# lucidrains/nuwa-pytorch

Hardware: AMD Instinct MI355X
Metric: video-tokens/sec, 3DNA decoder fwd+bwd @ 10x16x16 (higher is better)
Workload: dtype bf16/fp16 operands, fp32 accumulate -- forward: 3-MFMA bf16 hi+lo pairs on cross-attention kv projection, to_logits; 2 fp16 MFMAs (fp16 activation x fp16 hi+lo weight) on to_out x2, cross-attention q projection; single fp16 MFMA on 3DNA q/k/v projection, FF1 + gate, FF2, Sparse3DNA core, cross-atten

## Files before the change

nuwa_pytorch_amd/csrc/elementwise.hip:

```cpp
#include "common.h"
#include "../../include/amdnuwa.h"

namespace {

constexpr int MAXV = 4;
constexpr int ROWS_PER_BLOCK = 4;

template <int NV> struct RowValsT { float4 v[NV]; };
typedef RowValsT<MAXV> RowVals;

template <bool BF>
__device__ __forceinline__ float4 ld4(const void* base, size_t i) {
    if (BF) {
        const uint2 v = *reinterpret_cast<const uint2*>(reinterpret_cast<const bf16_t*>(base) + i);
        return make_float4(__uint_as_float(v.x << 16), __uint_as_float(v.x & 0xffff0000u), __uint_as_float(v.y << 16), __uint_as_float(v.y & 0xffff0000u));
    }
    return *reinterpret_cast<const float4*>(reinterpret_cast<const float*>(base) + i);
}
__device__ __forceinline__ float4 ld4h(const void* base, size_t i) {
    const uint2 v = *reinterpret_cast<const uint2*>(reinterpret_cast<const uint16_t*>(base) + i);
    return make_float4(f16lo_f(v.x), f16hi_f(v.x), f16lo_f(v.y), f16hi_f(v.y));
}
template <int FMT>
__device__ __forceinline__ float4 ld4f(const void* base, size_t i) {
    if constexpr (FMT == 2) return ld4h(base, i);
    else return ld4<FMT == 1>(base, i);
}
template <int FMT, int NV>
__device__ __forceinline__ void row_load_f(const void* base, size_t row_off, int D, int lane, RowValsT<NV>& r, float mul = 1.f) {
#pragma unroll
    for (int it = 0; it < NV; ++it) {
        const int e = (lane + it * 64) * 4;
        const bool in = e < D;
        const float4 v = ld4f<FMT>(base, row_off + (in ? e : 0));
        r.v[it] = make_float4(in ? v.x * mul : 0.f, in ? v.y * mul : 0.f, in ? v.z * mul : 0.f, in ? v.w * mul : 0.f);
    }
}
template <bool BF, int NV>
__device__ __forceinline__ void row_load_t(const void* base, size_t row_off, int D, int lane, RowValsT<NV>& r, float fill = 0.f) {
#pragma unroll
    for (int it = 0; it < NV; ++it) {
        const int e = (lane + it * 64) * 4;
        const bool in = e < D;
        const float4 v = ld4<BF>(base, row_off + (in ? e : 0));
        r.v[it] = make_float4(in ? v.x : fill, in ? v.y : fill, in ? v.z : fill, in ? v.w : fill);
    }
}

typedef float f32x4v __attribute__((ext_vector_type(4)));
typedef uint32_t u32x2v __attribute__((ext_vector_type(2)));
template <bool BF>
__device__ __forceinline__ float4 ld4_nt(const void* base, size_t i) {
    if (BF) {
        const u32x2v v = __builtin_nontemporal_load(reinterpret_cast<const u32x2v*>(reinterpret_cast<const bf16_t*>(base) + i));
        return make_float4(__uint_as_float(v.x << 16), __uint_as_float(v.x & 0xffff0000u), __uint_as_float(v.y << 16), __uint_as_float(v.y & 0xffff0000u));
    }
    const f32x4v v = __builtin_nontemporal_load(reinterpret_cast<const f32x4v*>(reinterpret_cast<const float*>(base) + i));
    return make_float4(v.x, v.y, v.z, v.w);
}
__device__ __forceinline__ void st4_nt(float* p, float4 v) {
    const f32x4v t = {v.x, v.y, v.z, v.w};
    __builtin_nontemporal_store(t, reinterpret_cast<f32x4v*>(p));
}
__device__ __forceinline__ void st_bf16x4_nt(bf16_t* p, float a, float b, float c, float d) {
    const u32x2v t = {pack2_rne(a, b), pack2_rne(c, d)};
    __builtin_nontemporal_store(t, reinterpret_cast<u32x2v*>(p));
}

template <int NV>
__device__ __forceinline__ void row_load(const float* __restrict__ p, int D, int lane, RowValsT<NV>& r, float fill = 0.f) {
#pragma unroll
    for (int it = 0; it < NV; ++it) {
        const int e = (lane + it * 64) * 4;
        const bool in = e < D;
        const float4 v = *reinterpret_cast<const float4*>(p + (in ? e : 0));
        r.v[it] = make_float4(in ? v.x : fill, in ? v.y : fill, in ? v.z : fill, in ? v.w : fill);
    }
}
__device__ __forceinline__ float4 ldp4(const float* __restrict__ p, int e, int D) {
    const bool in = e < D;
    const float4 v = *reinterpret_cast<const float4*>(p + (in ? e : 0));
    return make_float4(in ? v.x : 0.f, in ? v.y : 0.f, in ? v.z : 0.f, in ? v.w : 0.f);
}
__device__ __forceinline__ void store_bf16x4(bf16_t* hi, bf16_t* lo, int e, float a, float b, float c, float d, int lo_f16 = 0, float* sat = nullptr) {
    float dummy = 0.f;
    float& mx = sat ? *sat : dummy;
    if (lo_f16 == 2) { *reinterpret_cast<uint2*>(hi + e) = make_uint2(pack2_f16_sat_n(a, b, mx), pack2_f16_sat_n(c, d, mx)); return; }
    if (!lo) { *reinterpret_cast<uint2*>(hi + e) = make_uint2(pack2_rne(a, b), pack2_rne(c, d)); return; }
    if (lo_f16) {
        *reinterpret_cast<uint2*>(hi + e) = make_uint2(pack2_rne(a, b), pack2_rne(c, d));
        *reinterpret_cast<uint2*>(lo + e) = make_uint2(pack2_f16_sat_n(a, b, mx), pack2_f16_sat_n(c, d, mx));
        return;
    }
    bf16_t h[4], l[4];
    f2bf_hilo(a, h[0], l[0]); f2bf_hilo(b, h[1], l[1]); f2bf_hilo(c, h[2], l[2]); f2bf_hilo(d, h[3], l[3]);
    *reinterpret_cast<uint2*>(hi + e) = make_uint2(pack2(h[0], h[1]), pack2(h[2], h[3]));
    if (lo) *reinterpret_cast<uint2*>(lo + e) = make_uint2(pack2(l[0], l[1]), pack2(l[2], l[3]));
}

__device__ __forceinline__ void store_ln_shifted(bf16_t* out_hi, bf16_t* out_lo, long long row, int e, int D, int shift_ntok,
                                                 int shift_fmap, float y0, float y1, float y2, float y3, int lo_f16 = 0, float* sat = nullptr) {
    long long drow = row;
    bool keep = true, zero_own = false;
    if (shift_ntok > 0 && shift_fmap < 0) {
        const int i = (int)(row % shift_ntok);
        if (e < (D >> 1)) { keep = i + 1 < shift_ntok; drow = row + 1; zero_own = i == 0; }
    } else if (shift_ntok > 0) {
        const int i = (int)(row % shift_ntok);
        const int qd = e < (D >> 2) ? 0 : (e < (D >> 1) ? 1 : 2);
        if (i > 0 && qd < 2) {
            const int p = i - 1, wq = p % shift_fmap, yq = (p / shift_fmap) % shift_fmap;
            if (qd == 0) { keep = yq + 1 < shift_fmap && i + shift_fmap < shift_ntok; drow = row + shift_fmap; zero_own = yq == 0; }
            else         { keep = wq + 1 < shift_fmap && i + 1 < shift_ntok;          drow = row + 1;          zero_own = wq == 0; }
        }
    }
    if (keep) store_bf16x4(out_hi + drow * D, out_lo ? out_lo + drow * D : nullptr, e, y0, y1, y2, y3, lo_f16, sat);
    if (zero_own) store_bf16x4(out_hi + row * D, out_lo ? out_lo + row * D : nullptr, e, 0.f, 0.f, 0.f, 0.f, lo_f16, sat);
}

template <int NV>
__device__ __forceinline__ void row_mean_rstd(const RowValsT<NV>& xv, int D, int lane, float eps, float& mean, float& rstd) {
// ... 189 lines not shown
            const float4 wv = ldp4(w, e, D);
            float4 xx = cur.xv.v[it];
            const float4 gg = cur.gv.v[it];
            if (STABLE) { xx.x *= ia; xx.y *= ia; xx.z *= ia; xx.w *= ia; }
            xh[it] = make_float4((xx.x - mean) * rstd, (xx.y - mean) * rstd, (xx.z - mean) * rstd, (xx.w - mean) * rstd);
            g[it] = make_float4(gg.x * wv.x, gg.y * wv.y, gg.z * wv.z, gg.w * wv.w);
            s1 += (g[it].x + g[it].y) + (g[it].z + g[it].w);
            s2 += (g[it].x * xh[it].x + g[it].y * xh[it].y) + (g[it].z * xh[it].z + g[it].w * xh[it].w);
            pw[it].x += gg.x * xh[it].x; pw[it].y += gg.y * xh[it].y; pw[it].z += gg.z * xh[it].z; pw[it].w += gg.w * xh[it].w;
            pb[it].x += gg.x; pb[it].y += gg.y; pb[it].z += gg.z; pb[it].w += gg.w;
        }
        const float m1 = wave_sum(s1) / D, m2 = wave_sum(s2) / D;
        const float sc = STABLE ? rstd * ia : rstd;
#pragma unroll
        for (int it = 0; it < NV; ++it) {
            const int e = (lane + it * 64) * 4;
            if (e >= D) continue;
            const float d0 = sc * (g[it].x - m1 - xh[it].x * m2), d1 = sc * (g[it].y - m1 - xh[it].y * m2);
            const float d2 = sc * (g[it].z - m1 - xh[it].z * m2), d3 = sc * (g[it].w - m1 - xh[it].w * m2);
            ps[it].x += d0; ps[it].y += d1; ps[it].z += d2; ps[it].w += d3;
            if (OUT == 0) {
                if (out_f16) store_bf16x4(dx_hi + row * D, nullptr, e, d0 * gout, d1 * gout, d2 * gout, d3 * gout, 2, &sat);
                else store_bf16x4(dx_hi + row * D, dx_lo ? dx_lo + row * D : nullptr, e, d0, d1, d2, d3);
            } else {
                const float4 o = cur.rv.v[it];
                *reinterpret_cast<float4*>(dx_acc + row * D + e) = make_float4(o.x + d0, o.y + d1, o.z + d2, o.w + d3);
            }
        }
    };
    for (; row < R; row += 2 * stride) {
        const bool m1 = row + stride < R;
        if (m1) load_row(row + stride, bufB);
        process(bufA, row);
        if (!m1) break;
        if (row + 2 * stride < R) load_row(row + 2 * stride, bufA);
        process(bufB, row + stride);
    }
    if (OUT == 0) f16_sat_commit(sat);
#pragma unroll
    for (int it = 0; it < NV; ++it) {
        const int e = (lane + it * 64) * 4;
        *reinterpret_cast<float4*>(&red[wv_][0][e]) = pw[it];
        *reinterpret_cast<float4*>(&red[wv_][1][e]) = pb[it];
        *reinterpret_cast<float4*>(&red[wv_][2][e]) = ps[it];
    }
    __syncthreads();
    for (int idx = threadIdx.x; idx < 3 * D; idx += 256) {
        const int k = idx / D, c = idx % D;
        partial[((size_t)blockIdx.x * 3 + k) * D + c] = ((red[0][k][c] + red[1][k][c]) + red[2][k][c]) + red[3][k][c];
    }
}

template <int NV, int BFM, int NT = 0>
__global__ __launch_bounds__(256) void ln_bwd_chain_kernel(const float* __restrict__ dh, const float* __restrict__ x,
                                                           const float* __restrict__ mean_i, const float* __restrict__ rstd_i,
                                                           const float* __restrict__ w, const float* __restrict__ gres,
                                                           float* __restrict__ dx_out, const float* __restrict__ yprev,
                                                           const float* __restrict__ meanp_i, const float* __restrict__ rstdp_i,
                                                           const float* __restrict__ wprev, bf16_t* __restrict__ dyp_hi,
                                                           bf16_t* __restrict__ dyp_lo, float* __restrict__ partA,
                                                           float* __restrict__ partB, long long R, int D, int shift_ntok,
                                                           int shift_fmap, const float* __restrict__ scale2, int out_f16) {
#pragma clang fp contract(off)
    constexpr bool BF = BFM == 1 || BFM == 2, YBF = BFM == 1;
    constexpr int DHF = BFM == 3 ? 2 : (BF ? 1 : 0);
    const float gin = BFM == 3 ? f16_gs_inv(scale2) : 1.f, gout = out_f16 ? f16_gs(scale2) : 1.f;
    float sat = 0.f;
    __shared__ float red[ROWS_PER_BLOCK][3][NV * 256];
    const int lane = threadIdx.x & 63, wv_ = __builtin_amdgcn_readfirstlane(threadIdx.x >> 6);
    float4 pwA[NV], pbA[NV], pwB[NV], pbB[NV], psB[NV];
#pragma unroll
    for (int it = 0; it < NV; ++it) pwA[it] = pbA[it] = pwB[it] = pbB[it] = psB[it] = make_float4(0.f, 0.f, 0.f, 0.f);
    const int quarter = D >> 2;
    const float4 zero4 = make_float4(0.f, 0.f, 0.f, 0.f);
    struct RowIn { RowValsT<NV> xv, gv, rv, yv; float mean, rstd, meanp, rstdp; };
    auto load_row = [&](long long row, RowIn& in) {
        if (NT & 2) {
#pragma unroll
            for (int it = 0; it < NV; ++it) { const int e = (lane + it * 64) * 4; in.xv.v[it] = e < D ? ld4_nt<false>(x, (size_t)row * D + e) : zero4; }
        } else row_load(x + row * D, D, lane, in.xv);
        if (shift_ntok > 0) {
            const int i = (int)(row % shift_ntok);
            long long src_h = -1, src_w = -1;
            const bool audio = shift_fmap < 0;
            if (audio) {
                if (i + 1 < shift_ntok) src_h = src_w = row + 1;
            } else if (i > 0) {
                const int p = i - 1, wq = p % shift_fmap, yq = (p / shift_fmap) % shift_fmap;
                if (yq < shift_fmap - 1 && i + shift_fmap < shift_ntok) src_h = row + shift_fmap;
                if (wq < shift_fmap - 1 && i + 1 < shift_ntok) src_w = row + 1;
            }
#pragma unroll
            for (int it = 0; it < NV; ++it) {
                const int e0 = (lane + it * 64) * 4;
                const bool inr = e0 < D;
                const int e = inr ? e0 : 0;
                long long src = row;
                if (i > 0 || audio) { if (e < quarter) src = src_h; else if (e < 2 * quarter) src = src_w; }
                const bool has = src >= 0 && inr;
                const size_t so = (size_t)(has ? src : row) * D + e;
                const float4 v = BFM == 3 ? ld4h(dh, so) : ((NT & 2) ? ld4_nt<BF>(dh, so) : ld4<BF>(dh, so));
                in.gv.v[it] = make_float4(has ? v.x : 0.f, has ? v.y : 0.f, has ? v.z : 0.f, has ? v.w : 0.f);
            }
        } else {
            if (BFM == 3) row_load_f<2>(dh, (size_t)row * D, D, lane, in.gv);
            else row_load_t<BF>(dh, (size_t)row * D, D, lane, in.gv);
        }
        if (NT & 2) {
#pragma unroll
            for (int it = 0; it < NV; ++it) {
                const int e = (lane + it * 64) * 4;
                in.rv.v[it] = e < D ? ld4_nt<false>(gres, (size_t)row * D + e) : zero4;
                in.yv.v[it] = e < D ? ld4_nt<YBF>(yprev, (size_t)row * D + e) : zero4;
            }
        } else {
            row_load(gres + row * D, D, lane, in.rv);
            row_load_t<YBF>(yprev, (size_t)row * D, D, lane, in.yv);
        }
        in.mean = mean_i[row]; in.rstd = rstd_i[row]; in.meanp = meanp_i[row]; in.rstdp = rstdp_i[row];
    };
    const long long stride = (long long)gridDim.x * ROWS_PER_BLOCK;
    long long row = (long long)blockIdx.x * ROWS_PER_BLOCK + wv_;
    RowIn bufA, bufB;
    if (row < R) load_row(row, bufA);
    auto process = [&](const RowIn& cur, long long row) {
        float s1 = 0.f, s2 = 0.f;
        float4 xh[NV], g[NV];
#pragma unroll
        for (int it = 0; it < NV; ++it) {
            const int e = (lane + it * 64) * 4;
            const float4 wv = ldp4(w, e, D);
            const float4 xx = cur.xv.v[it], gg = cur.gv.v[it];
            xh[it] = make_float4((xx.x - cur.mean) * cur.rstd, (xx.y - cur.mean) * cur.rstd, (xx.z - cur.mean) * cur.rstd, (xx.w - cur.mean) * cur.rstd);
            g[it] = make_float4(gg.x * wv.x, gg.y * wv.y, gg.z * wv.z, gg.w * wv.w);
            s1 += (g[it].x + g[it].y) + (g[it].z + g[it].w);
            s2 += (g[it].x * xh[it].x + g[it].y * xh[it].y) + (g[it].z * xh[it].z + g[it].w * xh[it].w);
            pwA[it].x += gg.x * xh[it].x; pwA[it].y += gg.y * xh[it].y; pwA[it].z += gg.z * xh[it].z; pwA[it].w += gg.w * xh[it].w;
            pbA[it].x += gg.x; pbA[it].y += gg.y; pbA[it].z += gg.z; pbA[it].w += gg.w;
        }
        const float m1 = wave_sum(s1) / D, m2 = wave_sum(s2) / D;
        float4 dx[NV];
#pragma unroll
        for (int it = 0; it < NV; ++it) {
            const int e = (lane + it * 64) * 4;
            if (e >= D) { dx[it] = zero4; continue; }
            const float4 o = cur.rv.v[it];
            const float rs = BFM == 3 ? cur.rstd * gin : cur.rstd;
            dx[it] = make_float4(o.x + rs * (g[it].x - m1 - xh[it].x * m2), o.y + rs * (g[it].y - m1 - xh[it].y * m2),
                                 o.z + rs * (g[it].z - m1 - xh[it].z * m2), o.w + rs * (g[it].w - m1 - xh[it].w * m2));
            if (NT & 1) st4_nt(dx_out + row * D + e, dx[it]); else *reinterpret_cast<float4*>(dx_out + row * D + e) = dx[it];
        }
        s1 = 0.f; s2 = 0.f;
#pragma unroll
        for (int it = 0; it < NV; ++it) {
            const int e = (lane + it * 64) * 4;
            const float4 wv = ldp4(wprev, e, D);
            const float4 yy = cur.yv.v[it], gg = dx[it];
            xh[it] = make_float4((yy.x - cur.meanp) * cur.rstdp, (yy.y - cur.meanp) * cur.rstdp, (yy.z - cur.meanp) * cur.rstdp, (yy.w - cur.meanp) * cur.rstdp);
            g[it] = make_float4(gg.x * wv.x, gg.y * wv.y, gg.z * wv.z, gg.w * wv.w);
            s1 += (g[it].x + g[it].y) + (g[it].z + g[it].w);
            s2 += (g[it].x * xh[it].x + g[it].y * xh[it].y) + (g[it].z * xh[it].z + g[it].w * xh[it].w);
            pwB[it].x += gg.x * xh[it].x; pwB[it].y += gg.y * xh[it].y; pwB[it].z += gg.z * xh[it].z; pwB[it].w += gg.w * xh[it].w;
            pbB[it].x += gg.x; pbB[it].y += gg.y; pbB[it].z += gg.z; pbB[it].w += gg.w;
        }
        const float n1 = wave_sum(s1) / D, n2 = wave_sum(s2) / D;
#pragma unroll
        for (int it = 0; it < NV; ++it) {
            const int e = (lane + it * 64) * 4;
            if (e >= D) continue;
            const float rp = cur.rstdp * gout;
            const float d0 = rp * (g[it].x - n1 - xh[it].x * n2), d1 = rp * (g[it].y - n1 - xh[it].y * n2);
            const float d2 = rp * (g[it].z - n1 - xh[it].z * n2), d3 = rp * (g[it].w - n1 - xh[it].w * n2);
            psB[it].x += d0; psB[it].y += d1; psB[it].z += d2; psB[it].w += d3;
            if (out_f16) store_bf16x4(dyp_hi + row * D, nullptr, e, d0, d1, d2, d3, 2, &sat);
            else if ((NT & 1) && !dyp_lo) st_bf16x4_nt(dyp_hi + row * D + e, d0, d1, d2, d3);
            else store_bf16x4(dyp_hi + row * D, dyp_lo ? dyp_lo + row * D : nullptr, e, d0, d1, d2, d3);
        }
    };
    for (; row < R; row += 2 * stride) {
        const bool m1 = row + stride < R;
        if (m1) load_row(row + stride, bufB);
        process(bufA, row);
        if (!m1) break;
        if (row + 2 * stride < R) load_row(row + 2 * stride, bufA);
        process(bufB, row + stride);
    }
    f16_sat_commit(sat);
    if (BFM == 3 || out_f16) {
        const float ginv = BFM == 3 ? gin : 1.f, goutinv = out_f16 ? f16_gs_inv(scale2) : 1.f;
#pragma unroll
        for (int it = 0; it < NV; ++it) {
            pwA[it].x *= ginv; pwA[it].y *= ginv; pwA[it].z *= ginv; pwA[it].w *= ginv;
            pbA[it].x *= ginv; pbA[it].y *= ginv; pbA[it].z *= ginv; pbA[it].w *= ginv;
            psB[it].x *= goutinv; psB[it].y *= goutinv; psB[it].z *= goutinv; psB[it].w *= goutinv;
        }
    }
    for (int pass = 0; pass < 2; ++pass) {
        __syncthreads();
#pragma unroll
        for (int it = 0; it < NV; ++it) {
            const int e = (lane + it * 64) * 4;
            *reinterpret_cast<float4*>(&red[wv_][0][e]) = pass ? pwB[it] : pwA[it];
            *reinterpret_cast<float4*>(&red[wv_][1][e]) = pass ? pbB[it] : pbA[it];
            *reinterpret_cast<float4*>(&red[wv_][2][e]) = pass ? psB[it] : make_float4(0.f, 0.f, 0.f, 0.f);
        }
        __syncthreads();
        float* part = pass ? partB : partA;
        for (int idx = threadIdx.x; idx < 3 * D; idx += 256) {
            const int k = idx / D, c = idx % D;
            part[((size_t)blockIdx.x * 3 + k) * D + c] = ((red[0][k][c] + red[1][k][c]) + red[2][k][c]) + red[3][k][c];
        }
    }
}

__global__ __launch_bounds__(256) void colsum_kernel(const float* __restrict__ x, float* __restrict__ partial, long long R, int D) {
    for (int c = threadIdx.x; c < D; c += blockDim.x) {
        float s = 0.f;
        for (long long r = blockIdx.x; r < R; r += gridDim.x) s += x[r * D + c];
        partial[(size_t)blockIdx.x * D + c] = s;
    }
}

__global__ __launch_bounds__(1024) void partial_reduce_kernel(const float* __restrict__ partial, int nblk, int nk, int D,
                                                              float* __restrict__ o0, float* __restrict__ o1, float* __restrict__ o2, int accumulate) {
    __shared__ float red[64][17];
    const int col = threadIdx.x & 15, rg = threadIdx.x >> 4;
    const int idx = blockIdx.x * 16 + col;
    float s = 0.f;
    if (idx < nk * D)
        for (int bidx = rg; bidx < nblk; bidx += 64 * 4) {
            float v[4];
#pragma unroll
            for (int u = 0; u < 4; ++u) {
                const int bu = bidx + 64 * u;
                const float t = partial[(size_t)(bu < nblk ? bu : 0) * nk * D + idx];
                v[u] = bu < nblk ? t : 0.f;
            }
#pragma unroll
            for (int u = 0; u < 4; ++u) s += v[u];
        }
    red[rg][col] = s;
    __syncthreads();
    if (rg == 0 && idx < nk * D) {
        float t = 0.f;
#pragma unroll
        for (int r = 0; r < 64; ++r) t += red[r][col];
        const int k = idx / D, c = idx % D;
        float* o = k == 0 ? o0 : (k == 1 ? o1 : o2);
        if (o) o[c] = accumulate ? o[c] + t : t;
    }
}

__device__ __forceinline__ float hl(const bf16_t* hi, const bf16_t* lo, size_t i) { return bf2f(hi[i]) + (lo ? bf2f(lo[i]) : 0.f); }

__global__ void geglu_fwd_generic_kernel(const bf16_t* __restrict__ u_hi, const bf16_t* __restrict__ u_lo,
                                 bf16_t* __restrict__ o_hi, bf16_t* __restrict__ o_lo, long long R, int FP) {
    const size_t total = (size_t)R * FP / 4;
    for (size_t t = (size_t)blockIdx.x * blockDim.x + threadIdx.x; t < total; t += (size_t)gridDim.x * blockDim.x) {
        const size_t row = (t * 4) / FP;
        const int c = (int)((t * 4) % FP);
        const size_t ia = row * 2 * FP + c, ig = ia + FP;
        float o[4];
#pragma unroll
        for (int k = 0; k < 4; ++k) o[k] = hl(u_hi, u_lo, ia + k) * gelu_f(hl(u_hi, u_lo, ig + k));
        store_bf16x4(o_hi + row * FP, o_lo ? o_lo + row * FP : nullptr, c, o[0], o[1], o[2], o[3]);
    }
}

__global__ void geglu_bwd_generic_kernel(const bf16_t* __restrict__ u_hi, const bf16_t* __restrict__ u_lo,
                                 const bf16_t* __restrict__ d_hi, const bf16_t* __restrict__ d_lo,
                                 bf16_t* __restrict__ du_hi, bf16_t* __restrict__ du_lo, long long R, int FP) {
    const size_t total = (size_t)R * FP / 4;
    for (size_t t = (size_t)blockIdx.x * blockDim.x + threadIdx.x; t < total; t += (size_t)gridDim.x * blockDim.x) {
        const size_t row = (t * 4) / FP;
        const int c = (int)((t * 4) % FP);
        const size_t ia = row * 2 * FP + c, ig = ia + FP, id = row * FP + c;
        float da[4], dg[4];
#pragma unroll
        for (int k = 0; k < 4; ++k) {
            const float a = hl(u_hi, u_lo, ia + k), g = hl(u_hi, u_lo, ig + k), d = hl(d_hi, d_lo, id + k);
            da[k] = d * gelu_f(g);
            dg[k] = d * a * gelu_grad_f(g);
        }
        store_bf16x4(du_hi + row * 2 * FP, du_lo ? du_lo + row * 2 * FP : nullptr, c, da[0], da[1], da[2], da[3]);
        store_bf16x4(du_hi + row * 2 * FP, du_lo ? du_lo + row * 2 * FP : nullptr, c + FP, dg[0], dg[1], dg[2], dg[3]);
    }
}

__device__ __forceinline__ void unpack8(const uint4& v, float* f) {
    const uint32_t w[4] = {v.x, v.y, v.z, v.w};
#pragma unroll
    for (int k = 0; k < 4; ++k) { f[2 * k] = __uint_as_float(w[k] << 16); f[2 * k + 1] = __uint_as_float(w[k] & 0xffff0000u); }
}
template <bool LO>
__device__ __forceinline__ void load8(const bf16_t* hi, const bf16_t* lo, size_t off, float* f) {
    unpack8(*reinterpret_cast<const uint4*>(hi + off), f);
    if (LO) {
        float l[8];
        unpack8(*reinterpret_cast<const uint4*>(lo + off), l);
#pragma unroll
        for (int k = 0; k < 8; ++k) f[k] += l[k];
    }
}
// ... 460 lines not shown
    const dim3 block(256);
    static int n_cu = 0;
    if (!n_cu) { int dev = 0; (void)hipGetDevice(&dev); (void)hipDeviceGetAttribute(&n_cu, hipDeviceAttributeMultiprocessorCount, dev); if (n_cu <= 0) n_cu = 256; }
#define LNB_OCC(OU, ST, NV_, IN_) do { int o_ = 0; if (hipOccupancyMaxActiveBlocksPerMultiprocessor(&o_, ln_bwd_kernel<OU, ST, NV_, IN_>, 256, 0) == hipSuccess && o_ > 0 && o_ * n_cu < nb) nb = o_ * n_cu; } while (0)
#define LNB_(OU, ST, NV_, IN_) do { LNB_OCC(OU, ST, NV_, IN_); hipLaunchKernelGGL((ln_bwd_kernel<OU, ST, NV_, IN_>), dim3(nb), block, 0, stream, dy, x, mean, rstd, inv_amax, w, dx_hi, dx_lo, dx_acc, dres, part, R, D, shift_ntok, shift_fmap, scale2, out_f16); } while (0)
#define LNB(OU, ST, NV_) do { if (in_kind == 1) LNB_(OU, ST, NV_, 1); else if (in_kind == 2) LNB_(OU, ST, NV_, 2); else if (in_kind == 3) LNB_(OU, ST, NV_, 3); else LNB_(OU, ST, NV_, 0); } while (0)
#define LNB_NV(OU, ST) do { if (D <= 256) LNB(OU, ST, 1); else if (D <= 512) LNB(OU, ST, 2); else LNB(OU, ST, 4); } while (0)
    if (dx_hi) { if (stable) LNB_NV(0, true); else LNB_NV(0, false); }
    else       { if (stable) LNB_NV(1, true); else LNB_NV(1, false); }
#undef LNB_NV
#undef LNB
#undef LNB_
#undef LNB_OCC
    LAUNCH_CHECK();
    hipLaunchKernelGGL(partial_reduce_kernel, dim3((3 * D + 15) / 16), dim3(1024), 0, stream, part, nb, 3, D, dw, db, dsum, accumulate);
    LAUNCH_CHECK();
    return AMDNUWA_OK;
}

extern "C" size_t amdnuwa_ln_bwd_chain_workspace_bytes(long long R, int D) { return 2 * amdnuwa_ln_bwd_workspace_bytes(R, D); }

extern "C" int amdnuwa_ln_bwd_chain(const void* dh, const float* x, const float* mean, const float* rstd, const float* w,
                                    const float* g, float* dx, float* dw, float* db, const void* y_prev, const float* mean_prev,
                                    const float* rstd_prev, const float* w_prev, uint16_t* dy_prev_hi, uint16_t* dy_prev_lo,
                                    float* dw_prev, float* db_prev, float* dsum_prev, long long R, int D, int shift_ntok,
                                    int shift_fmap, int inputs_bf16, void* workspace, size_t workspace_bytes, hipStream_t stream) {
    if (inputs_bf16 < 0 || inputs_bf16 > 2) return AMDNUWA_ERR_ARG;
    return amdnuwa_ln_bwd_chain_f16(dh, x, mean, rstd, w, g, dx, dw, db, y_prev, mean_prev, rstd_prev, w_prev, dy_prev_hi, dy_prev_lo, dw_prev,
                                    db_prev, dsum_prev, R, D, shift_ntok, shift_fmap, inputs_bf16, 0, nullptr, workspace, workspace_bytes, stream);
}

extern "C" int amdnuwa_ln_bwd_chain_f16(const void* dh, const float* x, const float* mean, const float* rstd, const float* w,
                                        const float* g, float* dx, float* dw, float* db, const void* y_prev, const float* mean_prev,
                                        const float* rstd_prev, const float* w_prev, uint16_t* dy_prev_hi, uint16_t* dy_prev_lo,
                                        float* dw_prev, float* db_prev, float* dsum_prev, long long R, int D, int shift_ntok,
                                        int shift_fmap, int inputs_bf16, int dy_prev_f16, const float* scale2, void* workspace,
                                        size_t workspace_bytes, hipStream_t stream) {
    const int out_f16 = dy_prev_f16 ? 1 : 0;
    if (out_f16 && dy_prev_lo) return AMDNUWA_ERR_ARG;
    if (!dh || !x || !mean || !rstd || !w || !g || !dx || !y_prev || !mean_prev || !rstd_prev || !w_prev || !dy_prev_hi)
        return AMDNUWA_ERR_ARG;
    if (D % 4 || D > MAXV * 256 || D <= 0) return AMDNUWA_ERR_ARG;
    if (shift_ntok > 0 && (shift_fmap == 0 || shift_fmap < -1 || D % 16)) return AMDNUWA_ERR_ARG;
    if (inputs_bf16 < 0 || inputs_bf16 > 3) return AMDNUWA_ERR_ARG;
    if (!workspace || workspace_bytes < amdnuwa_ln_bwd_chain_workspace_bytes(R, D)) return AMDNUWA_ERR_WORKSPACE;
    if (R <= 0) return AMDNUWA_OK;
    int nb = ln_bwd_blocks(R);
    float* partA = (float*)workspace;
    float* partB = partA + (size_t)ln_bwd_blocks(R) * 3 * D;
    static int n_cu = 0;
    if (!n_cu) { int dev = 0; (void)hipGetDevice(&dev); (void)hipDeviceGetAttribute(&n_cu, hipDeviceAttributeMultiprocessorCount, dev); if (n_cu <= 0) n_cu = 256; }
    const int nt = g_amdnuwa_tuning[11] & 3;
#define LBC__(NV_, BF_, NT_) do { int o_ = 0; if (hipOccupancyMaxActiveBlocksPerMultiprocessor(&o_, ln_bwd_chain_kernel<NV_, BF_, NT_>, 256, 0) == hipSuccess && o_ > 0 && o_ * n_cu < nb) nb = o_ * n_cu; \
        if (g_amdnuwa_tuning[12] > 0 && g_amdnuwa_tuning[12] * n_cu < nb) nb = g_amdnuwa_tuning[12] * n_cu; \
        hipLaunchKernelGGL((ln_bwd_chain_kernel<NV_, BF_, NT_>), dim3(nb), dim3(256), 0, stream, (const float*)dh, x, mean, rstd, w, g, dx, (const float*)y_prev, mean_prev, rstd_prev, w_prev, dy_prev_hi, dy_prev_lo, partA, partB, R, D, shift_ntok, shift_fmap, scale2, out_f16); } while (0)
#define LBC_(NV_, BF_) do { if (nt == 0) LBC__(NV_, BF_, 0); else if (nt == 1) LBC__(NV_, BF_, 1); else if (nt == 2) LBC__(NV_, BF_, 2); else LBC__(NV_, BF_, 3); } while (0)
#define LBC(NV_) do { if (inputs_bf16 == 1) LBC_(NV_, 1); else if (inputs_bf16 == 2) LBC_(NV_, 2); else if (inputs_bf16 == 3) LBC__(NV_, 3, 0); else LBC_(NV_, 0); } while (0)
    if (D <= 256) LBC(1); else if (D <= 512) LBC(2); else LBC(4);
#undef LBC
#undef LBC_
#undef LBC__
    LAUNCH_CHECK();
    hipLaunchKernelGGL(partial_reduce_kernel, dim3((2 * D + 15) / 16), dim3(1024), 0, stream, partA, nb, 3, D, dw, db, (float*)nullptr, 0);
    hipLaunchKernelGGL(partial_reduce_kernel, dim3((3 * D + 15) / 16), dim3(1024), 0, stream, partB, nb, 3, D, dw_prev, db_prev, dsum_prev, 0);
    LAUNCH_CHECK();
    return AMDNUWA_OK;
}

AMDNUWA_SAT_ACCESSOR(elementwise)

namespace {
__global__ __launch_bounds__(256) void hilo_to_f16_kernel(const bf16_t* __restrict__ hi, const bf16_t* __restrict__ lo, int ld_in,
                                                          uint16_t* __restrict__ out, int ld_out, long long R, int C) {
    const long long chunks = R * (C / 8);
    for (long long e = (long long)blockIdx.x * blockDim.x + threadIdx.x; e < chunks; e += (long long)gridDim.x * blockDim.x) {
        const long long r = e / (C / 8);
        const int c = (int)(e % (C / 8)) * 8;
        const uint4 a = *reinterpret_cast<const uint4*>(hi + r * ld_in + c);
        const uint4 b = lo ? *reinterpret_cast<const uint4*>(lo + r * ld_in + c) : make_uint4(0, 0, 0, 0);
        const uint32_t aw[4] = {a.x, a.y, a.z, a.w}, bw[4] = {b.x, b.y, b.z, b.w};
        uint32_t o[4];
#pragma unroll
        for (int k = 0; k < 4; ++k) o[k] = pack2_f16_sat(lo_f(aw[k]) + lo_f(bw[k]), hi_f(aw[k]) + hi_f(bw[k]));
        *reinterpret_cast<uint4*>(out + r * ld_out + c) = make_uint4(o[0], o[1], o[2], o[3]);
    }
}
}

extern "C" int amdnuwa_hilo_to_f16(const uint16_t* hi, const uint16_t* lo, int ld_in, uint16_t* out, int ld_out, long long R, int C,
                                   hipStream_t stream) {
    if (!hi || !out || C <= 0 || C % 8 || ld_in % 8 || ld_out % 8) return AMDNUWA_ERR_ARG;
    if (R <= 0) return AMDNUWA_OK;
    hipLaunchKernelGGL(hilo_to_f16_kernel, dim3(grid_for((size_t)R * (C / 8))), dim3(256), 0, stream, hi, lo, ld_in, out, ld_out, R, C);
    LAUNCH_CHECK();
    return AMDNUWA_OK;
}

extern "C" size_t amdnuwa_colsum_workspace_bytes(long long R, int D) { return (size_t)(R < 256 ? (R < 1 ? 1 : R) : 256) * D * sizeof(float); }

extern "C" int amdnuwa_colsum(const float* x, float* out, long long R, int D, int accumulate, void* workspace, size_t workspace_bytes, hipStream_t stream) {
    if (!x || !out || D <= 0) return AMDNUWA_ERR_ARG;
    if (!workspace || workspace_bytes < amdnuwa_colsum_workspace_bytes(R, D)) return AMDNUWA_ERR_WORKSPACE;
    if (R <= 0) return AMDNUWA_OK;
    const int nb = (int)(R < 256 ? R : 256);
    hipLaunchKernelGGL(colsum_kernel, dim3(nb), dim3(256), 0, stream, x, (float*)workspace, R, D);
    LAUNCH_CHECK();
    hipLaunchKernelGGL(partial_reduce_kernel, dim3((D + 15) / 16), dim3(1024), 0, stream, (const float*)workspace, nb, 1, D, out, (float*)nullptr, (float*)nullptr, accumulate);
    LAUNCH_CHECK();
    return AMDNUWA_OK;
}

extern "C" int amdnuwa_geglu_fwd(const uint16_t* u_hi, const uint16_t* u_lo, uint16_t* o_hi, uint16_t* o_lo, long long R, int FP, hipStream_t stream) {
    if (!u_hi || !o_hi || FP % 4) return AMDNUWA_ERR_ARG;
    if (R <= 0) return AMDNUWA_OK;
    const dim3 rg((unsigned)((R + ROWS_PER_BLOCK - 1) / ROWS_PER_BLOCK));
    if (FP % 8) hipLaunchKernelGGL(geglu_fwd_generic_kernel, dim3(grid_for((size_t)R * FP / 4)), dim3(256), 0, stream, u_hi, u_lo, o_hi, o_lo, R, FP);
    else if (u_lo && o_lo) hipLaunchKernelGGL((geglu_fwd_kernel<true>), rg, dim3(256), 0, stream, u_hi, u_lo, o_hi, o_lo, R, FP);
// ... 127 lines not shown
```

Measured before the change: 719,300.

## Cut register pressure in fused LayerNorm backward chain and merge partial reductions

Rewrites the chained LayerNorm backward kernel to use fewer registers. Four accumulators move from registers into per-wave shared memory, the weights are staged in LDS, inputs are buffered as raw packed bf16/fp16 and converted late, per-row stats are read with one load per lane and broadcast with readlane, and shift offsets are tracked incrementally. It also adds a launch-bounds occupancy hint, a default grid cap, and fuses the two partial-reduce launches into one. The trade is extra LDS traffic, added barriers, and fewer blocks, which may reduce parallelism.

```diff
diff --git a/nuwa_pytorch_amd/csrc/elementwise.hip b/nuwa_pytorch_amd/csrc/elementwise.hip
--- a/nuwa_pytorch_amd/csrc/elementwise.hip
+++ b/nuwa_pytorch_amd/csrc/elementwise.hip
@@ -67,6 +67,29 @@
     __builtin_nontemporal_store(t, reinterpret_cast<u32x2v*>(p));
 }
 
+template <int FMT> struct Raw4 { typedef float4 T; };
+template <> struct Raw4<1> { typedef uint2 T; };
+template <> struct Raw4<2> { typedef uint2 T; };
+template <int FMT, bool NTL = false>
+__device__ __forceinline__ typename Raw4<FMT>::T ld_raw(const void* base, size_t i) {
+    if constexpr (FMT == 0) {
+        if constexpr (NTL) {
+            const f32x4v v = __builtin_nontemporal_load(reinterpret_cast<const f32x4v*>(reinterpret_cast<const float*>(base) + i));
+            return make_float4(v.x, v.y, v.z, v.w);
+        } else return *reinterpret_cast<const float4*>(reinterpret_cast<const float*>(base) + i);
+    } else {
+        if constexpr (NTL) {
+            const u32x2v v = __builtin_nontemporal_load(reinterpret_cast<const u32x2v*>(reinterpret_cast<const uint16_t*>(base) + i));
+            return make_uint2(v.x, v.y);
+        } else return *reinterpret_cast<const uint2*>(reinterpret_cast<const uint16_t*>(base) + i);
+    }
+}
+template <int FMT>
+__device__ __forceinline__ float4 cvt_raw(const typename Raw4<FMT>::T& v) {
+    if constexpr (FMT == 0) return v;
+    else if constexpr (FMT == 1) return make_float4(__uint_as_float(v.x << 16), __uint_as_float(v.x & 0xffff0000u), __uint_as_float(v.y << 16), __uint_as_float(v.y & 0xffff0000u));
+    else return make_float4(f16lo_f(v.x), f16hi_f(v.x), f16lo_f(v.y), f16hi_f(v.y));
+}
 template <int NV>
 __device__ __forceinline__ void row_load(const float* __restrict__ p, int D, int lane, RowValsT<NV>& r, float fill = 0.f) {
 #pragma unroll
@@ -362,7 +385,7 @@
 }
 
 template <int NV, int BFM, int NT = 0>
-__global__ __launch_bounds__(256) void ln_bwd_chain_kernel(const float* __restrict__ dh, const float* __restrict__ x,
+__global__ __launch_bounds__(256, NV <= 2 ? 3 : 1) void ln_bwd_chain_kernel(const float* __restrict__ dh, const float* __restrict__ x,
                                                            const float* __restrict__ mean_i, const float* __restrict__ rstd_i,
                                                            const float* __restrict__ w, const float* __restrict__ gres,
                                                            float* __restrict__ dx_out, const float* __restrict__ yprev,
@@ -372,149 +395,185 @@
                                                            float* __restrict__ partB, long long R, int D, int shift_ntok,
                                                            int shift_fmap, const float* __restrict__ scale2, int out_f16) {
 #pragma clang fp contract(off)
-    constexpr bool BF = BFM == 1 || BFM == 2, YBF = BFM == 1;
+    constexpr bool BF = BFM == 1 || BFM == 2, YBF = BFM == 1, NTL = (NT & 2) != 0;
     constexpr int DHF = BFM == 3 ? 2 : (BF ? 1 : 0);
+    constexpr int YF = YBF ? 1 : 0;
     const float gin = BFM == 3 ? f16_gs_inv(scale2) : 1.f, gout = out_f16 ? f16_gs(scale2) : 1.f;
     float sat = 0.f;
     __shared__ float red[ROWS_PER_BLOCK][3][NV * 256];
     const int lane = threadIdx.x & 63, wv_ = __builtin_amdgcn_readfirstlane(threadIdx.x >> 6);
-    float4 pwA[NV], pbA[NV], pwB[NV], pbB[NV], psB[NV];
-#pragma unroll
-    for (int it = 0; it < NV; ++it) pwA[it] = pbA[it] = pwB[it] = pbB[it] = psB[it] = make_float4(0.f, 0.f, 0.f, 0.f);
+    __shared__ float w_s[NV * 256], wp_s[NV * 256];
+    for (int c = threadIdx.x; c < NV * 256; c += 256) { w_s[c] = c < D ? w[c] : 0.f; wp_s[c] = c < D ? wprev[c] : 0.f; }
+    __shared__ float red_a[ROWS_PER_BLOCK][NV * 256];
+    float4 pwA[NV];
+#pragma unroll
+    for (int it = 0; it < NV; ++it) {
+        pwA[it] = make_float4(0.f, 0.f, 0.f, 0.f);
+        *reinterpret_cast<float4*>(&red_a[wv_][(lane + it * 64) * 4]) = make_float4(0.f, 0.f, 0.f, 0.f);
+#pragma unroll
+        for (int k = 0; k < 3; ++k) *reinterpret_cast<float4*>(&red[wv_][k][(lane + it * 64) * 4]) = make_float4(0.f, 0.f, 0.f, 0.f);
+    }
+    __syncthreads();
     const int quarter = D >> 2;
     const float4 zero4 = make_float4(0.f, 0.f, 0.f, 0.f);
-    struct RowIn { RowValsT<NV> xv, gv, rv, yv; float mean, rstd, meanp, rstdp; };
-    auto load_row = [&](long long row, RowIn& in) {
-        if (NT & 2) {
-#pragma unroll
-            for (int it = 0; it < NV; ++it) { const int e = (lane + it * 64) * 4; in.xv.v[it] = e < D ? ld4_nt<false>(x, (size_t)row * D + e) : zero4; }
-        } else row_load(x + row * D, D, lane, in.xv);
+    struct RowIn { float4 xv[NV], rv[NV]; typename Raw4<DHF>::T gv[NV]; typename Raw4<YF>::T yv[NV]; float st; int sh, sw; };
+    const float* const stat_p = lane == 0 ? mean_i : (lane == 1 ? rstd_i : (lane == 2 ? meanp_i : rstdp_i));
+    auto load_row = [&](long long row, int i, RowIn& in) {
+        int sh = 0, sw = 0;
         if (shift_ntok > 0) {
-            const int i = (int)(row % shift_ntok);
-            long long src_h = -1, src_w = -1;
-            const bool audio = shift_fmap < 0;
-            if (audio) {
-                if (i + 1 < shift_ntok) src_h = src_w = row + 1;
+            if (shift_fmap < 0) {
+                sh = sw = i + 1 < shift_ntok ? 1 : -1;
             } else if (i > 0) {
                 const int p = i - 1, wq = p % shift_fmap, yq = (p / shift_fmap) % shift_fmap;
-                if (yq < shift_fmap - 1 && i + shift_fmap < shift_ntok) src_h = row + shift_fmap;
-                if (wq < shift_fmap - 1 && i + 1 < shift_ntok) src_w = row + 1;
+                sh = (yq < shift_fmap - 1 && i + shift_fmap < shift_ntok) ? shift_fmap : -1;
+                sw = (wq < shift_fmap - 1 && i + 1 < shift_ntok) ? 1 : -1;
             }
-#pragma unroll
-            for (int it = 0; it < NV; ++it) {
-                const int e0 = (lane + it * 64) * 4;
-                const bool inr = e0 < D;
-                const int e = inr ? e0 : 0;
-                long long src = row;
-                if (i > 0 || audio) { if (e < quarter) src = src_h; else if (e < 2 * quarter) src = src_w; }
-                const bool has = src >= 0 && inr;
-                const size_t so = (size_t)(has ? src : row) * D + e;
-                const float4 v = BFM == 3 ? ld4h(dh, so) : ((NT & 2) ? ld4_nt<BF>(dh, so) : ld4<BF>(dh, so));
-                in.gv.v[it] = make_float4(has ? v.x : 0.f, has ? v.y : 0.f, has ? v.z : 0.f, has ? v.w : 0.f);
-            }
-        } else {
-            if (BFM == 3) row_load_f<2>(dh, (size_t)row * D, D, lane, in.gv);
-            else row_load_t<BF>(dh, (size_t)row * D, D, lane, in.gv);
-        }
-        if (NT & 2) {
-#pragma unroll
-            for (int it = 0; it < NV; ++it) {
-                const int e = (lane + it * 64) * 4;
-                in.rv.v[it] = e < D ? ld4_nt<false>(gres, (size_t)row * D + e) : zero4;
-                in.yv.v[it] = e < D ? ld4_nt<YBF>(yprev, (size_t)row * D + e) : zero4;
-            }
-        } else {
-            row_load(gres + row * D, D, lane, in.rv);
-            row_load_t<YBF>(yprev, (size_t)row * D, D, lane, in.yv);
-        }
-        in.mean = mean_i[row]; in.rstd = rstd_i[row]; in.meanp = meanp_i[row]; in.rstdp = rstdp_i[row];
+        }
+        in.sh = sh; in.sw = sw;
+        const size_t ro = (size_t)row * D;
+        const float* const xr = x + ro;
+        const float* const rr = gres + ro;
+        const void* const dr = DHF ? (const void*)(reinterpret_cast<const uint16_t*>(dh) + ro) : (const void*)(dh + ro);
+        const void* const yr = YF ? (const void*)(reinterpret_cast<const uint16_t*>(yprev) + ro) : (const void*)(yprev + ro);
+#pragma unroll
+        for (int it = 0; it < NV; ++it) { const int e0 = (lane + it * 64) * 4; in.xv[it] = ld_raw<0, NTL>(xr, (unsigned)(e0 < D ? e0 : 0)); }
+#pragma unroll
+        for (int it = 0; it < NV; ++it) {
+            const int e0 = (lane + it * 64) * 4;
+            const int e = e0 < D ? e0 : 0;
+            const int d = e < quarter ? sh : (e < 2 * quarter ? sw : 0);
+            in.gv[it] = ld_raw<DHF, NTL && BFM != 3>(dr, (unsigned)((d > 0 && e0 < D ? d * D : 0) + e));
+        }
+#pragma unroll
+        for (int it = 0; it < NV; ++it) { const int e0 = (lane + it * 64) * 4; in.rv[it] = ld_raw<0, NTL>(rr, (unsigned)(e0 < D ? e0 : 0)); }
+#pragma unroll
+        for (int it = 0; it < NV; ++it) { const int e0 = (lane + it * 64) * 4; in.yv[it] = ld_raw<YF, NTL>(yr, (unsigned)(e0 < D ? e0 : 0)); }
+        in.st = stat_p[row];
     };
-    const long long stride = (long long)gridDim.x * ROWS_PER_BLOCK;
-    long long row = (long long)blockIdx.x * ROWS_PER_BLOCK + wv_;
-    RowIn bufA, bufB;
-    if (row < R) load_row(row, bufA);
     auto process = [&](const RowIn& cur, long long row) {
+        const float cur_mean = __builtin_bit_cast(float, __builtin_amdgcn_readlane(__builtin_bit_cast(int, cur.st), 0));
+        const float cur_rstd = __builtin_bit_cast(float, __builtin_amdgcn_readlane(__builtin_bit_cast(int, cur.st), 1));
+        const float cur_meanp = __builtin_bit_cast(float, __builtin_amdgcn_readlane(__builtin_bit_cast(int, cur.st), 2));
+        const float cur_rstdp = __builtin_bit_cast(float, __builtin_amdgcn_readlane(__builtin_bit_cast(int, cur.st), 3));
         float s1 = 0.f, s2 = 0.f;
         float4 xh[NV], g[NV];
 #pragma unroll
         for (int it = 0; it < NV; ++it) {
-            const int e = (lane + it * 64) * 4;
-            const float4 wv = ldp4(w, e, D);
-            const float4 xx = cur.xv.v[it], gg = cur.gv.v[it];
-            xh[it] = make_float4((xx.x - cur.mean) * cur.rstd, (xx.y - cur.mean) * cur.rstd, (xx.z - cur.mean) * cur.rstd, (xx.w - cur.mean) * cur.rstd);
+            const int e0 = (lane + it * 64) * 4;
+            const bool inr = e0 < D;
+            const int e = inr ? e0 : 0;
+            const int d = e < quarter ? cur.sh : (e < 2 * quarter ? cur.sw : 0);
+            const bool has = d >= 0 && inr;
+            const float4 wv = *reinterpret_cast<const float4*>(w_s + e0);
+            const float4 xr = cur.xv[it], gr = cvt_raw<DHF>(cur.gv[it]);
+            const float4 xx = make_float4(inr ? xr.x : 0.f, inr ? xr.y : 0.f, inr ? xr.z : 0.f, inr ? xr.w : 0.f);
+            const float4 gg = make_float4(has ? gr.x : 0.f, has ? gr.y : 0.f, has ? gr.z : 0.f, has ? gr.w : 0.f);
+            xh[it] = make_float4((xx.x - cur_mean) * cur_rstd, (xx.y - cur_mean) * cur_rstd, (xx.z - cur_mean) * cur_rstd, (xx.w - cur_mean) * cur_rstd);
             g[it] = make_float4(gg.x * wv.x, gg.y * wv.y, gg.z * wv.z, gg.w * wv.w);
             s1 += (g[it].x + g[it].y) + (g[it].z + g[it].w);
             s2 += (g[it].x * xh[it].x + g[it].y * xh[it].y) + (g[it].z * xh[it].z + g[it].w * xh[it].w);
             pwA[it].x += gg.x * xh[it].x; pwA[it].y += gg.y * xh[it].y; pwA[it].z += gg.z * xh[it].z; pwA[it].w += gg.w * xh[it].w;
-            pbA[it].x += gg.x; pbA[it].y += gg.y; pbA[it].z += gg.z; pbA[it].w += gg.w;
-        }
+            float4 pb = *reinterpret_cast<float4*>(&red_a[wv_][e0]);
+            pb.x += gg.x; pb.y += gg.y; pb.z += gg.z; pb.w += gg.w;
+            *reinterpret_cast<float4*>(&red_a[wv_][e0]) = pb;
+        }
+        __builtin_amdgcn_sched_barrier(0);
         const float m1 = wave_sum(s1) / D, m2 = wave_sum(s2) / D;
         float4 dx[NV];
 #pragma unroll
         for (int it = 0; it < NV; ++it) {
             const int e = (lane + it * 64) * 4;
             if (e >= D) { dx[it] = zero4; continue; }
-            const float4 o = cur.rv.v[it];
-            const float rs = BFM == 3 ? cur.rstd * gin : cur.rstd;
+            const float4 o = cur.rv[it];
+            const float rs = BFM == 3 ? cur_rstd * gin : cur_rstd;
             dx[it] = make_float4(o.x + rs * (g[it].x - m1 - xh[it].x * m2), o.y + rs * (g[it].y - m1 - xh[it].y * m2),
                                  o.z + rs * (g[it].z - m1 - xh[it].z * m2), o.w + rs * (g[it].w - m1 - xh[it].w * m2));
             if (NT & 1) st4_nt(dx_out + row * D + e, dx[it]); else *reinterpret_cast<float4*>(dx_out + row * D + e) = dx[it];
         }
+        __builtin_amdgcn_sched_barrier(0);
         s1 = 0.f; s2 = 0.f;
 #pragma unroll
         for (int it = 0; it < NV; ++it) {
-            const int e = (lane + it * 64) * 4;
-            const float4 wv = ldp4(wprev, e, D);
-            const float4 yy = cur.yv.v[it], gg = dx[it];
-            xh[it] = make_float4((yy.x - cur.meanp) * cur.rstdp, (yy.y - cur.meanp) * cur.rstdp, (yy.z - cur.meanp) * cur.rstdp, (yy.w - cur.meanp) * cur.rstdp);
+            const int e0 = (lane + it * 64) * 4;
+            const bool inr = e0 < D;
+            const float4 wv = *reinterpret_cast<const float4*>(wp_s + e0);
+            const float4 yr = cvt_raw<YF>(cur.yv[it]), gg = dx[it];
+            const float4 yy = make_float4(inr ? yr.x : 0.f, inr ? yr.y : 0.f, inr ? yr.z : 0.f, inr ? yr.w : 0.f);
+            xh[it] = make_float4((yy.x - cur_meanp) * cur_rstdp, (yy.y - cur_meanp) * cur_rstdp, (yy.z - cur_meanp) * cur_rstdp, (yy.w - cur_meanp) * cur_rstdp);
             g[it] = make_float4(gg.x * wv.x, gg.y * wv.y, gg.z * wv.z, gg.w * wv.w);
             s1 += (g[it].x + g[it].y) + (g[it].z + g[it].w);
             s2 += (g[it].x * xh[it].x + g[it].y * xh[it].y) + (g[it].z * xh[it].z + g[it].w * xh[it].w);
-            pwB[it].x += gg.x * xh[it].x; pwB[it].y += gg.y * xh[it].y; pwB[it].z += gg.z * xh[it].z; pwB[it].w += gg.w * xh[it].w;
-            pbB[it].x += gg.x; pbB[it].y += gg.y; pbB[it].z += gg.z; pbB[it].w += gg.w;
-        }
+            float4 pw = *reinterpret_cast<float4*>(&red[wv_][0][e0]), pb = *reinterpret_cast<float4*>(&red[wv_][1][e0]);
+            pw.x += gg.x * xh[it].x; pw.y += gg.y * xh[it].y; pw.z += gg.z * xh[it].z; pw.w += gg.w * xh[it].w;
+            pb.x += gg.x; pb.y += gg.y; pb.z += gg.z; pb.w += gg.w;
+            *reinterpret_cast<float4*>(&red[wv_][0][e0]) = pw;
+            *reinterpret_cast<float4*>(&red[wv_][1][e0]) = pb;
+        }
+        __builtin_amdgcn_sched_barrier(0);
         const float n1 = wave_sum(s1) / D, n2 = wave_sum(s2) / D;
 #pragma unroll
         for (int it = 0; it < NV; ++it) {
             const int e = (lane + it * 64) * 4;
             if (e >= D) continue;
-            const float rp = cur.rstdp * gout;
+            const float rp = cur_rstdp * gout;
             const float d0 = rp * (g[it].x - n1 - xh[it].x * n2), d1 = rp * (g[it].y - n1 - xh[it].y * n2);
             const float d2 = rp * (g[it].z - n1 - xh[it].z * n2), d3 = rp * (g[it].w - n1 - xh[it].w * n2);
-            psB[it].x += d0; psB[it].y += d1; psB[it].z += d2; psB[it].w += d3;
+            float4 ps = *reinterpret_cast<float4*>(&red[wv_][2][e]);
+            ps.x += d0; ps.y += d1; ps.z += d2; ps.w += d3;
+            *reinterpret_cast<float4*>(&red[wv_][2][e]) = ps;
             if (out_f16) store_bf16x4(dyp_hi + row * D, nullptr, e, d0, d1, d2, d3, 2, &sat);
             else if ((NT & 1) && !dyp_lo) st_bf16x4_nt(dyp_hi + row * D + e, d0, d1, d2, d3);
             else store_bf16x4(dyp_hi + row * D, dyp_lo ? dyp_lo + row * D : nullptr, e, d0, d1, d2, d3);
         }
     };
-    for (; row < R; row += 2 * stride) {
-        const bool m1 = row + stride < R;
-        if (m1) load_row(row + stride, bufB);
-        process(bufA, row);
-        if (!m1) break;
-        if (row + 2 * stride < R) load_row(row + 2 * stride, bufA);
-        process(bufB, row + stride);
+    const long long stride = (long long)gridDim.x * ROWS_PER_BLOCK;
+    long long r0 = (long long)blockIdx.x * ROWS_PER_BLOCK + wv_;
+    if (r0 < R) {
+        const int istep = shift_ntok > 0 ? (int)(stride % shift_ntok) : 0;
+        int i0 = shift_ntok > 0 ? (int)(r0 % shift_ntok) : 0;
+        auto step = [&](const RowIn& cur, RowIn& fill) -> bool {
+            const long long r1 = r0 + stride;
+            const int i1 = i0 + istep >= shift_ntok ? i0 + istep - shift_ntok : i0 + istep;
+            const bool more = r1 < R;
+            load_row(more ? r1 : r0, more ? i1 : i0, fill);
+            __builtin_amdgcn_sched_barrier(0);
+            process(cur, r0);
+            r0 = r1; i0 = i1;
+            return !more;
+        };
+        RowIn bufA, bufB;
+        load_row(r0, i0, bufA);
+        while (!step(bufA, bufB) && !step(bufB, bufA)) {}
     }
     f16_sat_commit(sat);
-    if (BFM == 3 || out_f16) {
-        const float ginv = BFM == 3 ? gin : 1.f, goutinv = out_f16 ? f16_gs_inv(scale2) : 1.f;
+    if (BFM == 3) {
 #pragma unroll
         for (int it = 0; it < NV; ++it) {
-            pwA[it].x *= ginv; pwA[it].y *= ginv; pwA[it].z *= ginv; pwA[it].w *= ginv;
-            pbA[it].x *= ginv; pbA[it].y *= ginv; pbA[it].z *= ginv; pbA[it].w *= ginv;
-            psB[it].x *= goutinv; psB[it].y *= goutinv; psB[it].z *= goutinv; psB[it].w *= goutinv;
-        }
-    }
-    for (int pass = 0; pass < 2; ++pass) {
+            float4& pb = *reinterpret_cast<float4*>(&red_a[wv_][(lane + it * 64) * 4]);
+            pwA[it].x *= gin; pwA[it].y *= gin; pwA[it].z *= gin; pwA[it].w *= gin;
+            pb.x *= gin; pb.y *= gin; pb.z *= gin; pb.w *= gin;
+        }
+    }
+    if (out_f16) {
+        const float goutinv = f16_gs_inv(scale2);
+#pragma unroll
+        for (int it = 0; it < NV; ++it) {
+            float4& ps = *reinterpret_cast<float4*>(&red[wv_][2][(lane + it * 64) * 4]);
+            ps.x *= goutinv; ps.y *= goutinv; ps.z *= goutinv; ps.w *= goutinv;
+        }
+    }
+    for (int pass = 1; pass >= 0; --pass) {
         __syncthreads();
-#pragma unroll
-        for (int it = 0; it < NV; ++it) {
-            const int e = (lane + it * 64) * 4;
-            *reinterpret_cast<float4*>(&red[wv_][0][e]) = pass ? pwB[it] : pwA[it];
-            *reinterpret_cast<float4*>(&red[wv_][1][e]) = pass ? pbB[it] : pbA[it];
-            *reinterpret_cast<float4*>(&red[wv_][2][e]) = pass ? psB[it] : make_float4(0.f, 0.f, 0.f, 0.f);
-        }
-        __syncthreads();
+        if (pass == 0) {
+#pragma unroll
+            for (int it = 0; it < NV; ++it) {
+                const int e = (lane + it * 64) * 4;
+                *reinterpret_cast<float4*>(&red[wv_][0][e]) = pwA[it];
+                *reinterpret_cast<float4*>(&red[wv_][1][e]) = *reinterpret_cast<const float4*>(&red_a[wv_][e]);
+                *reinterpret_cast<float4*>(&red[wv_][2][e]) = make_float4(0.f, 0.f, 0.f, 0.f);
+            }
+            __syncthreads();
+        }
         float* part = pass ? partB : partA;
         for (int idx = threadIdx.x; idx < 3 * D; idx += 256) {
             const int k = idx / D, c = idx % D;
@@ -531,11 +590,11 @@
     }
 }
 
-__global__ __launch_bounds__(1024) void partial_reduce_kernel(const float* __restrict__ partial, int nblk, int nk, int D,
-                                                              float* __restrict__ o0, float* __restrict__ o1, float* __restrict__ o2, int accumulate) {
+__device__ __forceinline__ void partial_reduce_block(const float* __restrict__ partial, int nblk, int nk, int D, float* __restrict__ o0,
+                                                     float* __restrict__ o1, float* __restrict__ o2, int accumulate, int blk) {
     __shared__ float red[64][17];
     const int col = threadIdx.x & 15, rg = threadIdx.x >> 4;
-    const int idx = blockIdx.x * 16 + col;
+    const int idx = blk * 16 + col;
     float s = 0.f;
     if (idx < nk * D)
         for (int bidx = rg; bidx < nblk; bidx += 64 * 4) {
@@ -559,6 +618,17 @@
         float* o = k == 0 ? o0 : (k == 1 ? o1 : o2);
         if (o) o[c] = accumulate ? o[c] + t : t;
     }
+}
+__global__ __launch_bounds__(1024) void partial_reduce_kernel(const float* __restrict__ partial, int nblk, int nk, int D,
+                                                              float* __restrict__ o0, float* __restrict__ o1, float* __restrict__ o2, int accumulate) {
+    partial_reduce_block(partial, nblk, nk, D, o0, o1, o2, accumulate, blockIdx.x);
+}
+__global__ __launch_bounds__(1024) void partial_reduce_pair_kernel(const float* __restrict__ part_a, const float* __restrict__ part_b, int nblk,
+                                                                   int D, int blocks_a, float* __restrict__ a0, float* __restrict__ a1,
+                                                                   float* __restrict__ b0, float* __restrict__ b1, float* __restrict__ b2) {
+    const int first = (int)blockIdx.x < blocks_a;
+    partial_reduce_block(first ? part_a : part_b, nblk, 3, D, first ? a0 : b0, first ? a1 : b1, first ? (float*)nullptr : b2, 0,
+                         first ? (int)blockIdx.x : (int)blockIdx.x - blocks_a);
 }
 
 __device__ __forceinline__ float hl(const bf16_t* hi, const bf16_t* lo, size_t i) { return bf2f(hi[i]) + (lo ? bf2f(lo[i]) : 0.f); }
@@ -1125,7 +1195,8 @@
     if (!n_cu) { int dev = 0; (void)hipGetDevice(&dev); (void)hipDeviceGetAttribute(&n_cu, hipDeviceAttributeMultiprocessorCount, dev); if (n_cu <= 0) n_cu = 256; }
     const int nt = g_amdnuwa_tuning[11] & 3;
 #define LBC__(NV_, BF_, NT_) do { int o_ = 0; if (hipOccupancyMaxActiveBlocksPerMultiprocessor(&o_, ln_bwd_chain_kernel<NV_, BF_, NT_>, 256, 0) == hipSuccess && o_ > 0 && o_ * n_cu < nb) nb = o_ * n_cu; \
-        if (g_amdnuwa_tuning[12] > 0 && g_amdnuwa_tuning[12] * n_cu < nb) nb = g_amdnuwa_tuning[12] * n_cu; \
+        const int cap_ = g_amdnuwa_tuning[12] > 0 ? g_amdnuwa_tuning[12] : (NV_ == 1 ? 2 : 1); \
+        if (cap_ * n_cu < nb) nb = cap_ * n_cu; \
         hipLaunchKernelGGL((ln_bwd_chain_kernel<NV_, BF_, NT_>), dim3(nb), dim3(256), 0, stream, (const float*)dh, x, mean, rstd, w, g, dx, (const float*)y_prev, mean_prev, rstd_prev, w_prev, dy_prev_hi, dy_prev_lo, partA, partB, R, D, shift_ntok, shift_fmap, scale2, out_f16); } while (0)
 #define LBC_(NV_, BF_) do { if (nt == 0) LBC__(NV_, BF_, 0); else if (nt == 1) LBC__(NV_, BF_, 1); else if (nt == 2) LBC__(NV_, BF_, 2); else LBC__(NV_, BF_, 3); } while (0)
 #define LBC(NV_) do { if (inputs_bf16 == 1) LBC_(NV_, 1); else if (inputs_bf16 == 2) LBC_(NV_, 2); else if (inputs_bf16 == 3) LBC__(NV_, 3, 0); else LBC_(NV_, 0); } while (0)
@@ -1134,8 +1205,8 @@
 #undef LBC_
 #undef LBC__
     LAUNCH_CHECK();
-    hipLaunchKernelGGL(partial_reduce_kernel, dim3((2 * D + 15) / 16), dim3(1024), 0, stream, partA, nb, 3, D, dw, db, (float*)nullptr, 0);
-    hipLaunchKernelGGL(partial_reduce_kernel, dim3((3 * D + 15) / 16), dim3(1024), 0, stream, partB, nb, 3, D, dw_prev, db_prev, dsum_prev, 0);
+    const int blocks_a = (2 * D + 15) / 16, blocks_b = (3 * D + 15) / 16;
+    hipLaunchKernelGGL(partial_reduce_pair_kernel, dim3(blocks_a + blocks_b), dim3(1024), 0, stream, partA, partB, nb, D, blocks_a, dw, db, dw_prev, db_prev, dsum_prev);
     LAUNCH_CHECK();
     return AMDNUWA_OK;
 }
```

Result: no change. 716,200 (-0.4%).
